# KamilSJaron/smudgeplot

Measured on NVIDIA H100. Metric: k-mers/sec scanned (hetmers) at 1/2/4/8 H100; bit-exact .smu vs ref C, higher is better.
Workload: dtype u64

## Files before the change

smudgeplot_b200/csrc/hm_symm.cu:

```cuda
#include <cuda_runtime.h>
#include <stdint.h>
#include <stdio.h>
#include <stdlib.h>
#include <string.h>

#include "hetmers_b200.h"
#include "hm_internal.h"
#include "hm_device.cuh"

#define RS_THREADS 256
#define RS_EPT     8
#define RS_TILE    (RS_THREADS*RS_EPT)
#define RS_HALO    64
#define RS_WIN     (RS_TILE+2*RS_HALO)
#define RS_SCANCAP RS_HALO
#define RS_RUNCAP  (RS_HALO+1)
#define RS_LONGRUN 32
#ifndef RS_MINBLOCKS
#define RS_MINBLOCKS 5
#endif
#ifndef RS_STAGE
#define RS_STAGE   384
#endif

#define SY_STATUS_ASYMMETRIC 1ull
#define SY_STATUS_OVERFLOW   2ull

#define SY_HDR_CAND   0
#define SY_HDR_STATUS 1
#define SY_HDR_RUNS   2
#define SY_HDR_S      3
#define SY_HDR_PEND   4
#define SY_HDR_QUERY  5

struct SymmView
  { unsigned long long *cand_n;
    unsigned long long *status;
    uint32_t *bloom;
    uint32_t  seg_words;
    int       n_seg, self;
    uint64_t  first_key[HM_MAX_SHARDS];
    uint64_t *cand_key, *cand_lo, *cand_meta;
    unsigned long long cand_cap;
    unsigned long long *runs_n;
    uint64_t *runs;
    unsigned long long runs_cap;
    uint64_t *s_key, *s_lo;
    unsigned long long s_cap;
    const hm_stream_sview *sviews;
    uint64_t *pend, *pend_key, *pend_lo;
    uint64_t *q_key, *q_lo, *q_tag;
    unsigned long long pend_cap, q_cap;
  };

template <int KW>
__device__ __forceinline__ void bloom_slot(const SymmView &W, int seg, int kmer, uint64_t hi, uint64_t lo,
                                           uint32_t *&word, uint32_t &mask)
{ const int Pr = kmer >> 1, pup = kmer-Pr;
  uint64_t sfx;
  if (KW == 1)
    sfx = hi >> (64-2*kmer);
  else
    { const int sr = 128-2*kmer;
      sfx = sr == 0 ? lo : ((lo >> sr) | (hi << (64-sr)));
    }
  if (2*Pr < 64)
    sfx &= (((uint64_t) 1 << (2*Pr)) - 1);
  const uint64_t pfx = hi >> (64-2*pup);
  uint32_t h = ((uint32_t) sfx ^ (uint32_t) (sfx >> 32) * 0x85EBCA6Bu) * 0x9E3779B1u;
  uint32_t g = ((uint32_t) pfx ^ (uint32_t) (pfx >> 32) * 0xC2B2AE35u) * 0x27D4EB2Fu;
  h ^= h >> 15;
  word = W.bloom + (size_t) seg * W.seg_words + __umulhi(h * 0x2C1B3C6Du,W.seg_words);
  mask = (1u << (g >> 27)) | (1u << ((g >> 22) & 31));
}

__device__ __forceinline__ uint32_t ld_keep(const uint32_t *p)
{ uint32_t v; uint64_t pol;
  asm volatile("createpolicy.fractional.L2::evict_last.b64 %0, 1.0;" : "=l"(pol));
  asm volatile("ld.global.nc.L1::no_allocate.L2::cache_hint.u32 %0, [%1], %2;" : "=r"(v) : "l"(p), "l"(pol));
  return v;
}

__device__ __forceinline__ uint64_t ld_stream(const uint64_t *p)
{ uint64_t v, pol;
  asm volatile("createpolicy.fractional.L2::evict_first.b64 %0, 1.0;" : "=l"(pol));
  asm volatile("ld.global.nc.L1::no_allocate.L2::cache_hint.u64 %0, [%1], %2;" : "=l"(v) : "l"(p), "l"(pol));
  return v;
}

__device__ __forceinline__ int owner_of(const SymmView &W, uint64_t hi)
{ int r = 0;
  for (int s = 1; s < W.n_seg; s++)
    r += (hi >= W.first_key[s]);
  return r;
}

template <typename IdxT, int KW>
__device__ __noinline__ void neighbours_slow(const uint64_t *__restrict__ keys, const uint64_t *__restrict__ keys_lo,
                                             const uint16_t *__restrict__ cnt, const IdxT *__restrict__ bucket,
                                             int bshift, int kmer, int p0, int pup,
                                             uint64_t x, uint64_t xl, int cx,
                                             int &H, int &U, int64_t &part, int &ppos)
{ H = 0; U = 0; part = -1; ppos = 0;
  for (int p = p0; p < kmer; p++)
    { int b = base_at<KW>(x,xl,p);
      for (int c = 0; c < 4; c++)
        { if (c == b) continue;
          uint64_t y = x, yl = xl;
          set_base<KW>(y,yl,p,c);
          int64_t j = bucket_find<IdxT,KW>(keys,keys_lo,bucket,bshift,y,yl);
          if (j >= 0 && cx + (int) __ldg(cnt+j) <= HM_SMAX)
            { H += 1;
              if (p >= pup) U += 1;
              part = j; ppos = p;
            }
        }
    }
}


__device__ __forceinline__ uint64_t fp_mix(uint64_t hi, uint64_t lo, uint32_t c, uint64_t seed)
{ uint64_t v = (hi ^ seed) * 0xBF58476D1CE4E5B9ull;
  v ^= v >> 32;
  v = (v + lo + ((uint64_t) c << 40) + c) * 0x94D049BB133111EBull;
  v ^= v >> 29;
  v *= (seed | 1);
  v ^= v >> 32;
  return v;
}

template <int KW>
__global__ void __launch_bounds__(256)
symm_fingerprint_kernel(const uint64_t *__restrict__ keys, const uint64_t *__restrict__ keys_lo,
                        const uint16_t *__restrict__ cnt, int64_t i0, int64_t i1, int kmer,
                        uint64_t seed0, uint64_t seed1, unsigned long long *__restrict__ acc)
{ uint64_t a0 = 0, a1 = 0, a2 = 0, a3 = 0;
  const int64_t stride = (int64_t) gridDim.x * blockDim.x;
  for (int64_t i = i0 + (int64_t) blockIdx.x * blockDim.x + threadIdx.x; i < i1; i += stride)
    { uint64_t x = keys[i], xl = KW == 2 ? keys_lo[i] : 0, r, rl;
      uint32_t c = cnt[i];
      revcomp_kmer<KW>(x,xl,kmer,r,rl);
      a0 += fp_mix(x,xl,c,seed0);  a1 += fp_mix(x,xl,c,seed1);
      a2 += fp_mix(r,rl,c,seed0);  a3 += fp_mix(r,rl,c,seed1);
    }
  for (int o = 16; o > 0; o >>= 1)
    { a0 += __shfl_xor_sync(0xffffffffu,a0,o); a1 += __shfl_xor_sync(0xffffffffu,a1,o);
      a2 += __shfl_xor_sync(0xffffffffu,a2,o); a3 += __shfl_xor_sync(0xffffffffu,a3,o);
    }
  if ((threadIdx.x & 31) == 0)
    { atomicAdd(acc+0,(unsigned long long) a0); atomicAdd(acc+1,(unsigned long long) a1);
      atomicAdd(acc+2,(unsigned long long) a2); atomicAdd(acc+3,(unsigned long long) a3);
    }
}

extern "C" int hm_k_symm_fingerprint(const uint64_t *d_keys, const uint64_t *d_keys_lo, const uint16_t *d_cnt,
                                     int64_t i0, int64_t i1, int kmer, const uint64_t seed[2],
                                     uint64_t *d_acc, void *stream)
{ if (kmer < 1 || kmer > HM_MAX_KMER || (kmer > 32) != (d_keys_lo != NULL) || seed == NULL || d_acc == NULL)
    return hm_set_error(HM_EINVAL,"symm_fingerprint: bad arguments (k=%d)",kmer);
  if (i1 <= i0)
    return HM_OK;
  int64_t want = (i1-i0+255)/256;
  int     grid = (int) (want < 132*16 ? want : 132*16);
  if (kmer <= 32)
    symm_fingerprint_kernel<1><<<grid,256,0,(cudaStream_t) stream>>>
        (d_keys,NULL,d_cnt,i0,i1,kmer,seed[0],seed[1],(unsigned long long *) d_acc);
  else
    symm_fingerprint_kernel<2><<<grid,256,0,(cudaStream_t) stream>>>
        (d_keys,d_keys_lo,d_cnt,i0,i1,kmer,seed[0],seed[1],(unsigned long long *) d_acc);
  cudaError_t e = cudaGetLastError();
  if (e != cudaSuccess)
    return hm_cuda_fail(e,"symm_fingerprint_kernel");
  return HM_OK;
}

extern "C" void hm_symm_seeds(uint64_t seed[2])
// ... 236 lines not shown
                      int Hy, Uy, py; int64_t party;
                      neighbours_slow<IdxT,KW>(keys,keys_lo,cnt,bucket,bshift,kmer,Pr,pup,y,yl,cy,Hy,Uy,party,py);
                      if (Hy == 1)
                        { emit = true;
                          meta = pack_meta(cx,cy,ppos,base_at<KW>(y,yl,ppos));
                        }
                    }
                }
              const unsigned eb = __ballot_sync(FULL,emit);
              if (eb != 0)
                { unsigned long long base = 0;
                  if (lane == 0)
                    base = atomicAdd(W.cand_n,(unsigned long long) __popc(eb));
                  base = __shfl_sync(FULL,base,0) + (unsigned long long) __popc(eb & lt);
                  if (emit)
                    { if (base < W.cand_cap)
                        { W.cand_key[base] = x;
                          if (KW == 2) W.cand_lo[base] = xl;
                          W.cand_meta[base] = meta;
                        }
                      else
                        atomicOr(W.status,SY_STATUS_OVERFLOW);
                    }
                }
            }
        }
    }
}

template <int KW> struct RunSfx    { typedef uint64_t T; };
template <>       struct RunSfx<1> { typedef uint32_t T; };

template <int KW>
__device__ __forceinline__ typename RunSfx<KW>::T run_sfx(uint64_t hi, uint64_t lo, int Pr)
{ if constexpr (KW == 1)
    return (uint32_t) ((hi << 2*Pr) >> 32);
  else
    return (hi << (2*Pr-32) << 32) | (lo >> (64-2*Pr));
}

template <typename T>
__device__ __forceinline__ bool one_base_in_run(T d, int Pr, int &pos)
{ const T u = (d | (d >> 1)) & (T) HM_M5;
  if constexpr (sizeof(T) == 4) pos = Pr + (__clz((int) d) >> 1);
  else                          pos = Pr + (__clzll((long long) d) >> 1);
  return (u & (u-1)) == 0;
}

template <int KW, bool SL, int LMAX>
__device__ __forceinline__ bool settle_members(const RsSmem<KW> &S, const SymmView &W, int kmer, int Pr, int pup,
                                               int h, int L, int a, bool in, bool own, int lane,
                                               uint64_t &x, uint64_t &xl, uint64_t &meta)
{ int Hx = 0, Ux = 0, part = 0, ppos = 0, cx = 0;
  if (in)
    { x  = S.key[h+a];
      xl = KW == 2 ? S.klo[h+a] : 0;
      cx = S.cnt[h+a];
      auto mate = [&](int b)
        { int pos;
          if (b < L && b != a && one_base_in_run(run_sfx<KW>(x ^ S.key[h+b],KW == 2 ? xl ^ S.klo[h+b] : 0,Pr),Pr,pos) &&
              cx + (int) S.cnt[h+b] <= HM_SMAX)
            { Hx += 1;
              if (pos >= pup) Ux += 1;
              part = b; ppos = pos;
            }
        };
      if constexpr (LMAX > 0)
        {
#pragma unroll
          for (int b = 0; b < LMAX; b++)
            mate(b);
        }
      else
        for (int b = 0; b < L; b++)
          mate(b);
      if (own && Ux > 0)
        bloom_insert<KW,SL>(W,kmer,x,xl);
    }
  const int pl = lane + part - a;
  int       Hy = __shfl_sync(0xffffffffu,Hx,pl & 31);
  if (!in || !own || Hx != 1 || part < a)
    return false;
  const uint64_t y = S.key[h+part], yl = KW == 2 ? S.klo[h+part] : 0;
  const int      cy = S.cnt[h+part];
  if (pl > 31)
    { Hy = 0;
      for (int b = 0; b < L; b++)
        { int pos;
          if (b != part && one_base_in_run(run_sfx<KW>(y ^ S.key[h+b],KW == 2 ? yl ^ S.klo[h+b] : 0,Pr),Pr,pos) &&
              cy + (int) S.cnt[h+b] <= HM_SMAX)
            Hy += 1;
        }
    }
  if (Hy != 1)
    return false;
  meta = pack_meta(cx,cy,ppos,base_at<KW>(y,yl,ppos));
  return true;
}

#ifdef RS_PROBE
#define RS_PHASES 6
#define RS_PROBE_SLOTS 1024
__device__ unsigned long long rs_probe_cycles[RS_PROBE_SLOTS*RS_PHASES];
__device__ int rs_probe_mode;
#define RS_PROBE_TILE(b)  (rs_probe_mode == 2 ? (b) % 64 : (b))
#define RS_PROBE_START    long long rs_t = clock64(); unsigned long long rs_acc[RS_PHASES] = {0, 0, 0, 0, 0, 0};
#define RS_PROBE_MARK(ph) { const long long t_ = clock64(); rs_acc[ph] += (unsigned long long) (t_ - rs_t); rs_t = t_; }
#define RS_PROBE_FLUSH()  { if (lane == 0) _Pragma("unroll") for (int p_ = 0; p_ < RS_PHASES; p_++) \
                              atomicAdd(rs_probe_cycles + (blockIdx.x % RS_PROBE_SLOTS)*RS_PHASES + p_,rs_acc[p_]); }
#define RS_PROBE_LOADONLY() if (rs_probe_mode == 1) { RS_PROBE_FLUSH(); return; }

extern "C" int hm_probe_runscan(int mode, unsigned long long *cycles)
{ static unsigned long long rows[RS_PROBE_SLOTS*RS_PHASES];
  cudaError_t e = cudaDeviceSynchronize();
  if (e == cudaSuccess && cycles != NULL)
    { e = cudaMemcpyFromSymbol(rows,rs_probe_cycles,sizeof(rows));
      for (int p = 0; p < RS_PHASES; p++)
        { cycles[p] = 0;
          for (int r = 0; r < RS_PROBE_SLOTS; r++)
            cycles[p] += rows[r*RS_PHASES+p];
        }
    }
  memset(rows,0,sizeof(rows));
  if (e == cudaSuccess)
    e = cudaMemcpyToSymbol(rs_probe_cycles,rows,sizeof(rows));
  if (e == cudaSuccess)
    e = cudaMemcpyToSymbol(rs_probe_mode,&mode,sizeof(mode));
  return e == cudaSuccess ? HM_OK : hm_cuda_fail(e,"hm_probe_runscan");
}
#else
#define RS_PROBE_TILE(b)  (b)
#define RS_PROBE_START
#define RS_PROBE_MARK(ph)
#define RS_PROBE_FLUSH()
#define RS_PROBE_LOADONLY()
#endif

template <typename IdxT, int KW, bool SL>
__global__ void __launch_bounds__(RS_THREADS,RS_MINBLOCKS)
runscan_kernel(const uint64_t *__restrict__ keys, const uint64_t *__restrict__ keys_lo,
               const uint16_t *__restrict__ cnt, int64_t n, const IdxT *__restrict__ bucket, int bshift,
               int kmer, int64_t lo, int64_t hi, int64_t tile0, int use_tma, const SymmView W)
{ extern __shared__ __align__(128) uint8_t smem[];
  __shared__ __align__(8) uint64_t s_bar;
  __shared__ unsigned s_nc, s_nr, s_done;
  RsSmem<KW> S;
  S.key   = (uint64_t *) smem;
  S.klo   = S.key + (KW == 2 ? RS_WIN : 0);
  S.ckey  = S.key + KW*RS_WIN;
  S.clo   = S.ckey + (KW == 2 ? RS_STAGE : 0);
  S.cmeta = S.ckey + KW*RS_STAGE;
  S.cnt   = (uint16_t *) (S.cmeta + RS_STAGE);
  S.t1    = S.cnt + RS_WIN;
  S.t2r   = S.t1 + RS_TILE/2;

  const int      Pr   = kmer >> 1;
  const int      pup  = kmer - Pr;
  const int      psh  = 64-2*Pr;
  const uint64_t pmask = ~(uint64_t) 0 << psh;
  const unsigned FULL = 0xffffffffu;
  const int      lane = threadIdx.x & 31;
  const int      warp = threadIdx.x >> 5;
  const unsigned lt   = (1u << lane) - 1;
  RS_PROBE_START

  const int64_t T0 = (tile0 + RS_PROBE_TILE(blockIdx.x)) * RS_TILE;
  const int64_t ws = T0 - RS_HALO;
  const int64_t e0 = ws > 0 ? ws : 0;
  const int64_t e1 = T0+RS_TILE+RS_HALO < n ? T0+RS_TILE+RS_HALO : n;
  const int     v0 = (int) (e0-ws), v1 = (int) (e1-ws);

  const int m   = v1-v0;
  const int mt  = use_tma ? (m & ~7) : 0;
  if (threadIdx.x == 0)
    { s_nc = 0; s_nr = 0; s_done = 0;
      if (mt > 0)
        { mbar_init(&s_bar,1);
          fence_proxy_async_smem();
        }
    }
  __syncthreads();
  if (threadIdx.x == 0 && mt > 0)
    { mbar_arrive_expect_tx(&s_bar,(unsigned) (mt*(8*KW+2)));
      bulk_copy_g2s(S.key+v0,keys+e0,(unsigned) (8*mt),&s_bar);
      if (KW == 2)
        bulk_copy_g2s(S.klo+v0,keys_lo+e0,(unsigned) (8*mt),&s_bar);
      bulk_copy_g2s(S.cnt+v0,cnt+e0,(unsigned) (2*mt),&s_bar);
    }
  if (mt < m || v0 > 0 || v1 < RS_WIN)
    { for (int j = mt + threadIdx.x; j < m; j += RS_THREADS)
        { S.key[v0+j] = keys[e0+j];
          if (KW == 2) S.klo[v0+j] = keys_lo[e0+j];
          S.cnt[v0+j] = cnt[e0+j];
        }
      if (mt > 0)
        mbar_wait(&s_bar,0);
      __syncthreads();
      const uint64_t sa = ~S.key[v0], sb = ~S.key[v1-1];
      __syncthreads();
      for (int j = threadIdx.x; j < RS_WIN; j += RS_THREADS)
        if (j < v0)       S.key[j] = sa;
        else if (j >= v1) S.key[j] = sb;
      __syncthreads();
    }
  else
    mbar_wait(&s_bar,0);
  RS_PROBE_MARK(0)
  RS_PROBE_LOADONLY()

  const int wd0 = RS_HALO/32 + warp*RS_EPT;
  unsigned  eqw = 0;
#pragma unroll
  for (int t = 0; t < RS_EPT+2; t++)
    { const int i = (wd0-1+t)*32 + lane;
      bool eq;
      if (psh >= 32)
        { const uint32_t a = (uint32_t) (S.key[i] >> 32);
          uint32_t       b = __shfl_down_sync(FULL,a,1);
          if (lane == 31) b = (uint32_t) (S.key[i+1] >> 32);
          eq = (((a ^ b) >> (psh-32)) == 0);
        }
      else
        eq = (((S.key[i] ^ S.key[i+1]) & pmask) == 0);
      const unsigned bal = __ballot_sync(FULL,eq);
      if (lane == t) eqw = bal;
    }
  RS_PROBE_MARK(1)

  const int a0 = RS_HALO + (lo > T0 ? (int) (lo-T0 < RS_TILE ? lo-T0 : RS_TILE) : 0);
  const int a1 = RS_HALO + (hi-T0 < RS_TILE ? (int) (hi-T0) : RS_TILE);
  uint16_t *my1  = S.t1  + warp*(RS_TILE/2/(RS_THREADS/32));
  int n1, n3;
  { const unsigned P = __shfl_up_sync(FULL,eqw,1), N = __shfl_down_sync(FULL,eqw,1);
    unsigned m2 = 0, m3 = 0;
    const int wd = wd0-1+lane;
    if (lane >= 1 && lane <= RS_EPT)
      { const unsigned E = eqw;
        const unsigned em1 = (E << 1) | (P >> 31);
        const unsigned em2 = (E << 2) | (P >> 30);
        const unsigned ep1 = (E >> 1) | (N << 31);
        const int      s0  = wd*32;
        unsigned act = 0xffffffffu;
        if (s0 < a0)      act &= (a0-s0 >= 32) ? 0u : (0xffffffffu << (a0-s0));
        if (s0+32 > a1)   act &= (a1-s0 <= 0)  ? 0u : (0xffffffffu >> (s0+32-a1));
        const unsigned more = (em1 & E) | (E & ep1) | (em1 & em2);
        m2 = (E & ~em1 & ~ep1) & act;
        m3 = more & act & ~em1;
      }
    const int c2 = __popc(m2), c3 = __popc(m3);
    int pre2 = c2, pre3 = c3;
#pragma unroll
    for (int o = 1; o <= RS_EPT; o <<= 1)
      { int v2 = __shfl_up_sync(FULL,pre2,o), v3 = __shfl_up_sync(FULL,pre3,o);
        if (lane >= o) { pre2 += v2; pre3 += v3; }
      }
    n1 = __shfl_sync(FULL,pre2,RS_EPT);
    n3 = __shfl_sync(FULL,pre3,RS_EPT);
    int at = pre2-c2;
    while (m2 != 0)
      { my1[at++] = (uint16_t) (wd*32 + __ffs(m2)-1);
        m2 &= m2-1;
      }
    at = n1 + pre3-c3;
    while (m3 != 0)
      { my1[at++] = (uint16_t) (wd*32 + __ffs(m3)-1);
        m3 &= m3-1;
      }
  }
  __syncwarp();
  RS_PROBE_MARK(2)

  for (int i0 = 0; i0 < n1; i0 += 32)
    { const int i = i0+lane;
      bool     emit = false;
      uint64_t x = 0, xl = 0, meta = 0;
      if (i < n1)
        { const int w = my1[i];
          x = S.key[w];
          const uint64_t y = S.key[w+1];
          uint64_t yl = 0;
          if (KW == 2) { xl = S.klo[w]; yl = S.klo[w+1]; }
          const int cx = S.cnt[w], cy = S.cnt[w+1];
          int pos;
          if (one_base_in_run(run_sfx<KW>(x ^ y,xl ^ yl,Pr),Pr,pos) && cx+cy <= HM_SMAX)
            { emit = true;
              meta = pack_meta(cx,cy,pos,base_at<KW>(y,yl,pos));
              if (pos >= pup)
                { bloom_insert<KW,SL>(W,kmer,x,xl);
                  bloom_insert<KW,SL>(W,kmer,y,yl);
                }
            }
        }
      stage_candidates<KW>(S,&s_nc,W,emit,x,xl,meta,lane,lt);
    }
  RS_PROBE_MARK(3)

  const int b1 = hi-T0 < RS_TILE+RS_HALO ? RS_HALO + (int) (hi-T0) : RS_WIN;
  for (int i0 = 0; i0 < n3; i0 += 32)
    { const int i = i0+lane;
      const int h = i < n3 ? my1[n1+i] : 0;
      int       L = 0;
      {
        const int      t  = (h >> 5) - (wd0-1);
        const unsigned w0 = __shfl_sync(FULL,eqw,t & 31), w1 = __shfl_sync(FULL,eqw,(t+1) & 31);
        const unsigned up = __funnelshift_r(w0,w1,h & 31);
        if (i < n3)
          L = (~up != 0) ? __ffs((int) ~up) : 33;
      }
      const int Ls = L <= 8 ? L : 0;
      int inc = Ls;
#pragma unroll
      for (int o = 1; o < 32; o <<= 1)
        { const int v = __shfl_up_sync(FULL,inc,o);
          if (lane >= o) inc += v;
        }
      const int M = __shfl_sync(FULL,inc,31);
      for (int t0 = 0; t0 < M; t0 += 32)
        { const int t = t0+lane;
          int r = 0;
#pragma unroll
          for (int s = 16; s > 0; s >>= 1)
            if (__shfl_sync(FULL,inc,r+s-1) <= t) r += s;
          const int hr = __shfl_sync(FULL,h,r), Lr = __shfl_sync(FULL,Ls,r);
          const int a  = t - (__shfl_sync(FULL,inc,r) - Lr);
          bool     emit = false;
          uint64_t x = 0, xl = 0, meta = 0;
          emit = settle_members<KW,SL,8>(S,W,kmer,Pr,pup,hr,Lr,a,t < M,hr+a < b1,lane,x,xl,meta);
          stage_candidates<KW>(S,&s_nc,W,emit,x,xl,meta,lane,lt);
        }
      unsigned lb = __ballot_sync(FULL,L > 8);
      while (lb != 0)
        { const int src = __ffs(lb)-1;
          lb &= lb-1;
          const int hh = __shfl_sync(FULL,h,src);
          int       LL = __shfl_sync(FULL,L,src);
          if (LL > 32)
            { const uint64_t xh = S.key[hh];
              while (LL <= RS_RUNCAP)
                { const int      t = hh+LL+lane;
                  const unsigned sb = __ballot_sync(FULL,t < RS_WIN && ((S.key[t] ^ xh) & pmask) == 0);
                  if (sb != FULL) { LL += __ffs(~sb)-1; break; }
                  LL += 32;
                }
            }
          if (LL > RS_RUNCAP || hh+LL >= RS_WIN)
            { if (lane == 0)
                S.t2r[atomicAdd(&s_nr,1u)] = (uint16_t) hh;
              continue;
            }
          for (int a0 = 0; a0 < LL; a0 += 32)
            { const int a = a0+lane;
              bool     emit = false;
              uint64_t x = 0, xl = 0, meta = 0;
              emit = settle_members<KW,SL,0>(S,W,kmer,Pr,pup,hh,LL,a,a < LL,hh+a < b1,lane,x,xl,meta);
              stage_candidates<KW>(S,&s_nc,W,emit,x,xl,meta,lane,lt);
            }
        }
    }
  RS_PROBE_MARK(4)

  __syncwarp();
  unsigned last = 0;
  if (lane == 0)
    { __threadfence_block();
      last = (atomicAdd(&s_done,1u) == RS_THREADS/32-1);
    }
  last = __shfl_sync(FULL,last,0);
  if (!last)
    { RS_PROBE_MARK(5) RS_PROBE_FLUSH() return; }
  __threadfence_block();
  const unsigned nr = s_nr;
  if (nr > 0)
    { unsigned long long rb = 0;
      if (lane == 0)
        rb = atomicAdd(W.runs_n,(unsigned long long) nr);
      rb = __shfl_sync(FULL,rb,0);
      for (unsigned i = lane; i < nr; i += 32)
        if (rb+i < W.runs_cap)
          W.runs[rb+i] = (uint64_t) (T0 + ((int) S.t2r[i] - RS_HALO));
        else
          atomicOr(W.status,SY_STATUS_OVERFLOW);
    }
  const unsigned nc = s_nc < RS_STAGE ? s_nc : RS_STAGE;
  if (nc == 0)
    { RS_PROBE_MARK(5) RS_PROBE_FLUSH() return; }
  unsigned long long base = 0;
  if (lane == 0)
    base = atomicAdd(W.cand_n,(unsigned long long) nc);
  base = __shfl_sync(FULL,base,0);
  for (unsigned i = lane; i < nc; i += 32)
    { unsigned long long at = base + i;
      if (at < W.cand_cap)
        { W.cand_key[at] = S.ckey[i];
          if (KW == 2) W.cand_lo[at] = S.clo[i];
          W.cand_meta[at] = S.cmeta[i];
        }
      else
        atomicOr(W.status,SY_STATUS_OVERFLOW);
    }
  RS_PROBE_MARK(5)
  RS_PROBE_FLUSH()
}

template <typename IdxT, int KW, bool SL>
__global__ void __launch_bounds__(RS_THREADS,RS_MINBLOCKS)
runscan_dense_kernel(const uint64_t *__restrict__ keys, const uint64_t *__restrict__ keys_lo,
                     const uint16_t *__restrict__ cnt, int64_t n, int kmer, int64_t lo, int64_t hi,
                     int64_t tile0, int use_tma, const SymmView W)
{ extern __shared__ __align__(128) uint8_t smem[];
  __shared__ __align__(8) uint64_t s_bar;
  __shared__ unsigned s_nc, s_nl, s_done;
  __shared__ unsigned s_eq[RS_WIN/32+1];
  RsSmem<KW> S;
  S.key   = (uint64_t *) smem;
  S.klo   = S.key + (KW == 2 ? RS_WIN : 0);
  S.ckey  = S.key + KW*RS_WIN;
  S.clo   = S.ckey + (KW == 2 ? RS_STAGE : 0);
  S.cmeta = S.ckey + KW*RS_STAGE;
  S.cnt   = (uint16_t *) (S.cmeta + RS_STAGE);
  S.t1    = S.cnt + RS_WIN;
  S.t2r   = S.t1 + RS_WIN;
  uint16_t *s_part = S.t2r + RS_TILE/8;
  unsigned *hu = (unsigned *) (s_part + RS_WIN);
  uint32_t *rem = hu + RS_WIN/2;

  const int      Pr   = kmer >> 1, pup = kmer - Pr, psh = 64-2*Pr;
  const uint64_t pmask = ~(uint64_t) 0 << psh;
  const unsigned FULL = 0xffffffffu;
  const int      lane = threadIdx.x & 31;
  const int      warp = threadIdx.x >> 5;
  const unsigned lt   = (1u << lane) - 1;

  const int64_t T0 = (tile0 + blockIdx.x) * RS_TILE;
  const int64_t ws = T0 - RS_HALO;
  const int64_t e0 = ws > 0 ? ws : 0;
  const int64_t e1 = T0+RS_TILE+RS_HALO < n ? T0+RS_TILE+RS_HALO : n;
  const int     v0 = (int) (e0-ws), v1 = (int) (e1-ws);

  const int m   = v1-v0;
  const int mt  = use_tma ? (m & ~7) : 0;
  if (threadIdx.x == 0)
    { s_nc = 0; s_nl = 0; s_done = 0;
      if (mt > 0)
        { mbar_init(&s_bar,1);
          fence_proxy_async_smem();
        }
    }
  for (int j = threadIdx.x; j < RS_WIN/2; j += RS_THREADS)
    hu[j] = 0;
  __syncthreads();
  if (threadIdx.x == 0 && mt > 0)
    { mbar_arrive_expect_tx(&s_bar,(unsigned) (mt*(8*KW+2)));
      bulk_copy_g2s(S.key+v0,keys+e0,(unsigned) (8*mt),&s_bar);
      if (KW == 2)
        bulk_copy_g2s(S.klo+v0,keys_lo+e0,(unsigned) (8*mt),&s_bar);
      bulk_copy_g2s(S.cnt+v0,cnt+e0,(unsigned) (2*mt),&s_bar);
    }
  if (mt < m || v0 > 0 || v1 < RS_WIN)
    { for (int j = mt + threadIdx.x; j < m; j += RS_THREADS)
        { S.key[v0+j] = keys[e0+j];
          if (KW == 2) S.klo[v0+j] = keys_lo[e0+j];
          S.cnt[v0+j] = cnt[e0+j];
        }
      if (mt > 0)
        mbar_wait(&s_bar,0);
      __syncthreads();
      const uint64_t sa = ~S.key[v0], sb = ~S.key[v1-1];
      __syncthreads();
      for (int j = threadIdx.x; j < RS_WIN; j += RS_THREADS)
        if (j < v0)       S.key[j] = sa;
        else if (j >= v1) S.key[j] = sb;
      __syncthreads();
    }
  else
    mbar_wait(&s_bar,0);

  const bool narrow = (KW == 1) && (kmer-Pr <= 16);
  for (int wd = warp; wd < RS_WIN/32; wd += RS_THREADS/32)
    { const int i = wd*32 + lane;
      bool eq = false;
      const uint64_t ki = S.key[i];
      if (i+1 < RS_WIN)
        eq = (((ki ^ S.key[i+1]) & pmask) == 0);
// ... 20 lines not shown
          back = (~dn == 0) ? 32 : __clz((int) ~dn);
        }
      uint16_t mark = (uint16_t) fwd;
      if (back+fwd+1 > RS_LONGRUN)
        { mark = 0xffff;
          if (back == 0 && i >= a0 && i < a1)
            S.t2r[atomicAdd(&s_nl,1u)] = (uint16_t) i;
        }
      S.t1[i] = mark;
      s_part[i] = (uint16_t) i;
    }
  __syncthreads();

  for (int i = threadIdx.x; i < RS_WIN; i += RS_THREADS)
    { const int fwd = S.t1[i];
      if (fwd == 0 || fwd == 0xffff)
        continue;
      const int cx = S.cnt[i];
      if (narrow)
        { const uint32_t rx = rem[i];
          for (int j = i+1; j <= i+fwd; j++)
            { const uint32_t d = rx ^ rem[j];
              const uint32_t u = (d | (d>>1)) & 0x55555555u;
              if ((u & (u-1)) == 0 && cx + (int) S.cnt[j] <= HM_SMAX)
                { const int      pos = Pr + (__clz((int) d) >> 1);
                  const unsigned inc = 1u | (pos >= pup ? 0x100u : 0u);
                  atomicAdd(hu + (i>>1), inc << (16*(i&1)));
                  atomicAdd(hu + (j>>1), inc << (16*(j&1)));
                  s_part[i] = (uint16_t) j;
                  s_part[j] = (uint16_t) i;
                }
            }
        }
      else
        { const uint64_t x = S.key[i], xl = KW == 2 ? S.klo[i] : 0;
          for (int j = i+1; j <= i+fwd; j++)
            { int pos;
              if (one_base_apart<KW>(x,xl,S.key[j],KW == 2 ? S.klo[j] : 0,pos) && cx + (int) S.cnt[j] <= HM_SMAX)
                { const unsigned inc = 1u | (pos >= pup ? 0x100u : 0u);
                  atomicAdd(hu + (i>>1), inc << (16*(i&1)));
                  atomicAdd(hu + (j>>1), inc << (16*(j&1)));
                  s_part[i] = (uint16_t) j;
                  s_part[j] = (uint16_t) i;
                }
            }
        }
    }
  __syncthreads();

  for (int i0 = RS_HALO + (threadIdx.x & ~31); i0 < RS_HALO+RS_TILE; i0 += RS_THREADS)
    { const int i = i0+lane;
      bool     emit = false;
      uint64_t x = 0, xl = 0, meta = 0;
      if (i >= a0 && i < a1 && S.t1[i] != 0xffff)
        { const unsigned c = (hu[i>>1] >> (16*(i&1))) & 0xffffu;
          const int H = (int) (c & 0xff), U = (int) (c >> 8);
          if (H > 0)
            { x = S.key[i];
              if (KW == 2) xl = S.klo[i];
              if (U > 0)
                bloom_insert<KW,SL>(W,kmer,x,xl);
              const int j = s_part[i];
              if (H == 1 && j > i && ((hu[j>>1] >> (16*(j&1))) & 0xffu) == 1)
                { const uint64_t y = S.key[j], yl = KW == 2 ? S.klo[j] : 0;
                  int pos;
                  one_base_apart<KW>(x,xl,y,yl,pos);
                  emit = true;
                  meta = pack_meta(S.cnt[i],S.cnt[j],pos,base_at<KW>(y,yl,pos));
                }
            }
        }
      stage_candidates<KW>(S,&s_nc,W,emit,x,xl,meta,lane,lt);
    }

  __syncwarp();
  unsigned last = 0;
  if (lane == 0)
    { __threadfence_block();
      last = (atomicAdd(&s_done,1u) == RS_THREADS/32-1);
    }
  last = __shfl_sync(FULL,last,0);
  if (!last)
    return;
  __threadfence_block();
  const unsigned nr = s_nl;
  if (nr > 0)
    { unsigned long long rb = 0;
      if (lane == 0)
        rb = atomicAdd(W.runs_n,(unsigned long long) nr);
      rb = __shfl_sync(FULL,rb,0);
      for (unsigned i = lane; i < nr; i += 32)
        if (rb+i < W.runs_cap)
          W.runs[rb+i] = (uint64_t) (T0 + ((int) S.t2r[i] - RS_HALO));
        else
          atomicOr(W.status,SY_STATUS_OVERFLOW);
    }
  const unsigned nc = s_nc < RS_STAGE ? s_nc : RS_STAGE;
  if (nc == 0)
    return;
  unsigned long long base = 0;
  if (lane == 0)
    base = atomicAdd(W.cand_n,(unsigned long long) nc);
  base = __shfl_sync(FULL,base,0);
  for (unsigned i = lane; i < nc; i += 32)
    { unsigned long long at = base + i;
      if (at < W.cand_cap)
        { W.cand_key[at] = S.ckey[i];
          if (KW == 2) W.cand_lo[at] = S.clo[i];
          W.cand_meta[at] = S.cmeta[i];
        }
      else
        atomicOr(W.status,SY_STATUS_OVERFLOW);
    }
}

template <typename I, int K> struct Inst { typedef I IdxT; static constexpr int KW = K; };

template <class F>
static cudaError_t dispatch(int kmer, int idx64, F f)
{ if (kmer <= 32)
    return idx64 ? f(Inst<uint64_t,1>()) : f(Inst<uint32_t,1>());
  return idx64 ? f(Inst<uint64_t,2>()) : f(Inst<uint32_t,2>());
}

template <typename IdxT, int KW, bool SL = false>
static cudaError_t launch_runscan(const uint64_t *keys, const uint64_t *keys_lo, const uint16_t *cnt, int64_t n,
                                  const void *bucket, int bits, int kmer, int64_t lo, int64_t hi,
                                  const SymmView &W, cudaStream_t st)
{ static int configured[64] = {0};
  int dev = 0;
  cudaGetDevice(&dev);
  int64_t tile0 = lo/RS_TILE, tile1 = (hi+RS_TILE-1)/RS_TILE;
  int     tma   = ((((uintptr_t) keys) | ((uintptr_t) cnt) | ((uintptr_t) (keys_lo ? keys_lo : keys))) & 15) == 0;
  const int   Pr  = kmer >> 1;
  double      lam = (2*Pr >= 62) ? 0.0 : (double) n / (double) ((uint64_t) 1 << (2*Pr));
  bool        dense = (lam > 0.6);
  const char *force = getenv("HETMERS_RUNSCAN");
  if (force != NULL && strcmp(force,"dense") == 0)  dense = true;
  if (force != NULL && strcmp(force,"sparse") == 0) dense = false;
  cudaError_t e;
  if (dense)
    { size_t smem = (size_t) RS_WIN*(8*KW+2) + (size_t) RS_STAGE*8*(KW+1) +
                    2*(size_t) (RS_WIN+RS_TILE/8+RS_WIN) + 4*(size_t) (RS_WIN/2+RS_WIN);
      if (smem > 48*1024 && (dev >= 64 || !(configured[dev] & 2)))
        { e = cudaFuncSetAttribute(runscan_dense_kernel<IdxT,KW,SL>,cudaFuncAttributeMaxDynamicSharedMemorySize,(int) smem);
          if (e != cudaSuccess) return e;
          if (dev < 64) configured[dev] |= 2;
        }
      runscan_dense_kernel<IdxT,KW,SL><<<(unsigned) (tile1-tile0),RS_THREADS,smem,st>>>
          (keys,keys_lo,cnt,n,kmer,lo,hi,tile0,tma,W);
    }
  else
    { size_t smem = (size_t) RS_WIN*(8*KW+2) + (size_t) RS_STAGE*8*(KW+1) +
                    2*(size_t) (RS_TILE/2+RS_TILE/2);
      if (smem > 48*1024 && (dev >= 64 || !(configured[dev] & 1)))
        { e = cudaFuncSetAttribute(runscan_kernel<IdxT,KW,SL>,cudaFuncAttributeMaxDynamicSharedMemorySize,(int) smem);
          if (e != cudaSuccess) return e;
          if (dev < 64) configured[dev] |= 1;
        }
      runscan_kernel<IdxT,KW,SL><<<(unsigned) (tile1-tile0),RS_THREADS,smem,st>>>
          (keys,keys_lo,cnt,n,(const IdxT *) bucket,64-bits,kmer,lo,hi,tile0,tma,W);
    }
  return cudaGetLastError();
}

template <typename IdxT, int KW, bool SL = false>
static cudaError_t launch_runs(const uint64_t *keys, const uint64_t *keys_lo, const uint16_t *cnt, int64_t n,
                               const void *bucket, int bits, int kmer, int64_t lo, int64_t hi,
                               const SymmView &W, cudaStream_t st)
{
  int dev = 0, sms = 132;
  cudaGetDevice(&dev);
  cudaDeviceGetAttribute(&sms,cudaDevAttrMultiProcessorCount,dev);
  int64_t want = ((hi-lo)/64+255)/256;
  int     grid = (int) (want < sms*8 ? (want > 0 ? want : 1) : sms*8);
  runs_kernel<IdxT,KW,SL><<<grid,256,0,st>>>(keys,keys_lo,cnt,n,(const IdxT *) bucket,64-bits,kmer,lo,hi,W);
  return cudaGetLastError();
}

extern "C" int hm_k_symm_runscan(const uint64_t *d_keys, const uint64_t *d_keys_lo, const uint16_t *d_cnt, int64_t n,
                                 const void *d_bucket, int bits, int idx64, int kmer, int64_t lo, int64_t hi,
                                 void *d_work, const hm_symm_layout *layout, const hm_symm_shards *shards,
                                 void *stream)
{ if (kmer < HM_SYMM_MIN_KMER || kmer > HM_MAX_KMER)
    return hm_set_error(HM_EUNSUPPORTED,"symmetric scan needs %d <= k <= %d (k=%d)",HM_SYMM_MIN_KMER,HM_MAX_KMER,kmer);
  if (lo < 0 || hi > n || lo > hi || bits < 1 || bits > 30 || d_work == NULL || layout == NULL)
    return hm_set_error(HM_EINVAL,"symm_runscan: bad range [%lld,%lld) of %lld or bits %d",
                        (long long) lo,(long long) hi,(long long) n,bits);
  if ((kmer > 32) != (d_keys_lo != NULL))
    return hm_set_error(HM_EINVAL,"symm_runscan: second key word array %s for k=%d",
                        d_keys_lo ? "given" : "missing",kmer);
  if ((shards != NULL && shards->n_seg > 1) != (layout->n_seg > 1) ||
      (shards != NULL && shards->n_seg > 1 && (shards->n_seg != layout->n_seg || shards->self < 0 ||
                                               shards->self >= shards->n_seg)))
    return hm_set_error(HM_EINVAL,"symm_runscan: shard table does not match the work-area layout");
  cudaStream_t st = (cudaStream_t) stream;
  SymmView W = make_view(d_work,layout,shards);
  HM_CUDA(cudaMemsetAsync(W.cand_n,0,256,st));
  HM_CUDA(cudaMemsetAsync(W.bloom + (size_t) W.self*W.seg_words,0,sizeof(uint32_t)*(size_t) W.seg_words,st));
  if (l2_persist())
    bloom_window(st,W.bloom,sizeof(uint32_t)*(size_t) W.seg_words*(size_t) W.n_seg,1);
  if (hi == lo)
    return HM_OK;
  cudaError_t e = dispatch(kmer,idx64,[&](auto I)
    { return launch_runscan<typename decltype(I)::IdxT,decltype(I)::KW>(d_keys,d_keys_lo,d_cnt,n,d_bucket,bits,kmer,
                                                                       lo,hi,W,st); });
  if (e != cudaSuccess)
    return hm_cuda_fail(e,"runscan_kernel");
  return HM_OK;
}

extern "C" int hm_k_symm_runs(const uint64_t *d_keys, const uint64_t *d_keys_lo, const uint16_t *d_cnt, int64_t n,
                              const void *d_bucket, int bits, int idx64, int kmer, int64_t lo, int64_t hi,
                              void *d_work, const hm_symm_layout *layout, const hm_symm_shards *shards,
                              void *stream)
{ if (kmer < HM_SYMM_MIN_KMER || kmer > HM_MAX_KMER || d_work == NULL || layout == NULL ||
      (kmer > 32) != (d_keys_lo != NULL) || lo < 0 || hi > n || lo > hi)
    return hm_set_error(HM_EINVAL,"symm_runs: bad arguments");
  if (hi == lo)
    return HM_OK;
  cudaStream_t st = (cudaStream_t) stream;
  SymmView W = make_view(d_work,layout,shards);
  cudaError_t e = dispatch(kmer,idx64,[&](auto I)
    { return launch_runs<typename decltype(I)::IdxT,decltype(I)::KW>(d_keys,d_keys_lo,d_cnt,n,d_bucket,bits,kmer,
                                                                    lo,hi,W,st); });
  if (e != cudaSuccess)
    return hm_cuda_fail(e,"runs_kernel");
  return HM_OK;
}


#define RV_TS   192
#define RV_TM   96
#define RV_TROW 97
#define RV_THREADS 1024
#ifndef RV_ILP
#define RV_ILP 2
#endif
#define RV_QCAP  (32*(RV_ILP+1))
#define RV_PROBE 4
#define RV_HA    (1ull << 48)
#define RV_HB    (1ull << 49)

#ifdef RESOLVE_PROBE
#define RVP_BINS 50
#define RVP_CAND 0
#define RVP_HA   1
#define RVP_HB   2
#define RVP_HAB  3
#define RVP_GEN  4
#define RVP_HIST 5
#define RVP_NCTR (RVP_HIST+RVP_BINS)
__device__ unsigned long long rvp_ctr[RVP_NCTR];
__device__ int rvp_mode;
#define RVP_MODE rvp_mode
#define RVP_COUNT(i,v) { if (rvp_mode == 3) atomicAdd(rvp_ctr+(i),(unsigned long long) (v)); }
#define RVP_BUCKET(sz) RVP_COUNT(RVP_HIST + ((sz) < RVP_BINS-1 ? (int) (sz) : RVP_BINS-1),1)

extern "C" int hm_probe_resolve(int mode, unsigned long long *ctr)
{ static unsigned long long rows[RVP_NCTR];
  cudaError_t e = cudaDeviceSynchronize();
  if (e == cudaSuccess && ctr != NULL)
    { e = cudaMemcpyFromSymbol(rows,rvp_ctr,sizeof(rows));
      memcpy(ctr,rows,sizeof(rows));
    }
  memset(rows,0,sizeof(rows));
  if (e == cudaSuccess)
    e = cudaMemcpyToSymbol(rvp_ctr,rows,sizeof(rows));
  if (e == cudaSuccess)
    e = cudaMemcpyToSymbol(rvp_mode,&mode,sizeof(mode));
  return e == cudaSuccess ? HM_OK : hm_cuda_fail(e,"hm_probe_resolve");
}
#else
#define RVP_MODE 0
#define RVP_COUNT(i,v)
#define RVP_BUCKET(sz)
#endif

template <int KW>
__device__ __forceinline__ bool bucket_upper_partner(const uint64_t *__restrict__ keys, const uint64_t *__restrict__ keys_lo,
                                                     const uint16_t *__restrict__ cnt, int64_t l, int64_t r,
                                                     int psh, int pup, uint64_t q, uint64_t ql, int cq, bool &found)
{ bool hit = false;
  found = false;
  for (int64_t i0 = l; i0 < r; i0 += RV_PROBE)
    { uint64_t z[RV_PROBE];
#pragma unroll
      for (int u = 0; u < RV_PROBE; u++)
        z[u] = (i0+u < r) ? __ldg(keys+i0+u) : ~q;
#pragma unroll
      for (int u = 0; u < RV_PROBE; u++)
        { if (((z[u] ^ q) >> psh) != 0)
            continue;
          const uint64_t zl = KW == 2 ? __ldg(keys_lo+i0+u) : 0;
          int pos;
          if (z[u] == q && (KW == 1 || zl == ql))
            found = true;
          else if (one_base_apart<KW>(q,ql,z[u],zl,pos) && pos >= pup && cq + (int) __ldg(cnt+i0+u) <= HM_SMAX)
            hit = true;
        }
    }
  return hit;
}

template <typename IdxT, int KW>
__device__ __noinline__ bool has_upper_partner(const uint64_t *__restrict__ keys, const uint64_t *__restrict__ keys_lo,
                                               const uint16_t *__restrict__ cnt, int64_t n,
// ... 815 lines not shown
```

Before: 119.4 billion.

## Classify short runs by bitmask and emit members directly, skipping warp scan expansion

Run heads are now split with bit tricks into short runs (length at most 8) and long runs. Short runs have all their member positions written straight into the per-warp list through an add-carry fill mask, and each member recovers its run start and length from the eq bitmask with funnel shifts and clz/ffs. This removes the per-batch warp prefix scan and binary search that previously expanded short runs into members. Long runs are stored from the end of an enlarged per-warp list, the three counts are packed into one scan, and the list shared memory grows a little, which could affect occupancy.

```diff
diff --git a/smudgeplot_b200/csrc/hm_symm.cu b/smudgeplot_b200/csrc/hm_symm.cu
--- a/smudgeplot_b200/csrc/hm_symm.cu
+++ b/smudgeplot_b200/csrc/hm_symm.cu
@@ -22,6 +22,7 @@
 #ifndef RS_STAGE
 #define RS_STAGE   384
 #endif
+#define RS_WLIST   (RS_TILE/(RS_THREADS/32)+8)
 
 #define SY_STATUS_ASYMMETRIC 1ull
 #define SY_STATUS_OVERFLOW   2ull
@@ -564,7 +565,7 @@
   S.cmeta = S.ckey + KW*RS_STAGE;
   S.cnt   = (uint16_t *) (S.cmeta + RS_STAGE);
   S.t1    = S.cnt + RS_WIN;
-  S.t2r   = S.t1 + RS_TILE/2;
+  S.t2r   = S.t1 + RS_WLIST*(RS_THREADS/32);
 
   const int      Pr   = kmer >> 1;
   const int      pup  = kmer - Pr;
@@ -641,43 +642,54 @@
 
   const int a0 = RS_HALO + (lo > T0 ? (int) (lo-T0 < RS_TILE ? lo-T0 : RS_TILE) : 0);
   const int a1 = RS_HALO + (hi-T0 < RS_TILE ? (int) (hi-T0) : RS_TILE);
-  uint16_t *my1  = S.t1  + warp*(RS_TILE/2/(RS_THREADS/32));
-  int n1, n3;
+  uint16_t *my1  = S.t1  + warp*RS_WLIST;
+  int n1, nm, n9;
   { const unsigned P = __shfl_up_sync(FULL,eqw,1), N = __shfl_down_sync(FULL,eqw,1);
-    unsigned m2 = 0, m3 = 0;
-    const int wd = wd0-1+lane;
+    unsigned m2 = 0, m9 = 0, mlo = 0, mhi = 0;
     if (lane >= 1 && lane <= RS_EPT)
       { const unsigned E = eqw;
         const unsigned em1 = (E << 1) | (P >> 31);
         const unsigned em2 = (E << 2) | (P >> 30);
         const unsigned ep1 = (E >> 1) | (N << 31);
-        const int      s0  = wd*32;
+        const int      s0  = (wd0-1+lane)*32;
         unsigned act = 0xffffffffu;
         if (s0 < a0)      act &= (a0-s0 >= 32) ? 0u : (0xffffffffu << (a0-s0));
         if (s0+32 > a1)   act &= (a1-s0 <= 0)  ? 0u : (0xffffffffu >> (s0+32-a1));
         const unsigned more = (em1 & E) | (E & ep1) | (em1 & em2);
         m2 = (E & ~em1 & ~ep1) & act;
-        m3 = more & act & ~em1;
+        const unsigned m3 = more & act & ~em1;
+        const uint64_t X  = (uint64_t) E | ((uint64_t) N << 32);
+        uint64_t       c8 = X & (X >> 1);
+        c8 &= c8 >> 2;
+        c8 &= c8 >> 4;
+        m9 = m3 & (uint32_t) c8;
+        const uint64_t fill = (X + (m3 & ~(uint32_t) c8)) ^ X;
+        mlo = (uint32_t) fill;
+        mhi = (uint32_t) (fill >> 32);
       }
-    const int c2 = __popc(m2), c3 = __popc(m3);
-    int pre2 = c2, pre3 = c3;
+    const unsigned mm = mlo | __shfl_up_sync(FULL,mhi,1);
+    const unsigned c = __popc(m2) | (__popc(mm) << 10) | (__popc(m9) << 20);
+    unsigned pre = c;
 #pragma unroll
     for (int o = 1; o <= RS_EPT; o <<= 1)
-      { int v2 = __shfl_up_sync(FULL,pre2,o), v3 = __shfl_up_sync(FULL,pre3,o);
-        if (lane >= o) { pre2 += v2; pre3 += v3; }
+      { const unsigned v = __shfl_up_sync(FULL,pre,o);
+        if (lane >= o) pre += v;
       }
-    n1 = __shfl_sync(FULL,pre2,RS_EPT);
-    n3 = __shfl_sync(FULL,pre3,RS_EPT);
-    int at = pre2-c2;
-    while (m2 != 0)
-      { my1[at++] = (uint16_t) (wd*32 + __ffs(m2)-1);
-        m2 &= m2-1;
-      }
-    at = n1 + pre3-c3;
-    while (m3 != 0)
-      { my1[at++] = (uint16_t) (wd*32 + __ffs(m3)-1);
-        m3 &= m3-1;
-      }
+    const unsigned tot = __shfl_sync(FULL,pre,RS_EPT+1);
+    n1 = tot & 1023;
+    nm = (tot >> 10) & 1023;
+    n9 = tot >> 20;
+    pre -= c;
+    const int s0 = (wd0-1+lane)*32;
+    int at = pre & 1023;
+    for (unsigned b = m2; b != 0; b &= b-1)
+      my1[at++] = (uint16_t) (s0 + __ffs(b)-1);
+    at = n1 + ((pre >> 10) & 1023);
+    for (unsigned b = mm; b != 0; b &= b-1)
+      my1[at++] = (uint16_t) (s0 + __ffs(b)-1);
+    at = RS_WLIST-1 - (int) (pre >> 20);
+    for (unsigned b = m9; b != 0; b &= b-1)
+      my1[at--] = (uint16_t) (s0 + __ffs(b)-1);
   }
   __syncwarp();
   RS_PROBE_MARK(2)
@@ -708,39 +720,32 @@
   RS_PROBE_MARK(3)
 
   const int b1 = hi-T0 < RS_TILE+RS_HALO ? RS_HALO + (int) (hi-T0) : RS_WIN;
-  for (int i0 = 0; i0 < n3; i0 += 32)
+  for (int i0 = 0; i0 < nm; i0 += 32)
+    { const int      i  = i0+lane;
+      const int      s  = i < nm ? my1[n1+i] : wd0*32;
+      const int      tq = ((s-1) >> 5) - (wd0-1), ts = (s >> 5) - (wd0-1);
+      const unsigned q0 = __shfl_sync(FULL,eqw,(tq-1) & 31), q1 = __shfl_sync(FULL,eqw,tq & 31);
+      const unsigned w0 = __shfl_sync(FULL,eqw,ts & 31),     w1 = __shfl_sync(FULL,eqw,(ts+1) & 31);
+      const unsigned dn = __funnelshift_l(q0,q1,31-((s-1) & 31));
+      const unsigned up = __funnelshift_r(w0,w1,s & 31);
+      const int      a  = __clz((int) ~dn), L = a + __ffs((int) ~up);
+      bool     emit = false;
+      uint64_t x = 0, xl = 0, meta = 0;
+      emit = settle_members<KW,SL,8>(S,W,kmer,Pr,pup,s-a,L,a,i < nm,s < b1,lane,x,xl,meta);
+      stage_candidates<KW>(S,&s_nc,W,emit,x,xl,meta,lane,lt);
+    }
+  for (int i0 = 0; i0 < n9; i0 += 32)
     { const int i = i0+lane;
-      const int h = i < n3 ? my1[n1+i] : 0;
+      const int h = i < n9 ? my1[RS_WLIST-1-i] : 0;
       int       L = 0;
       {
         const int      t  = (h >> 5) - (wd0-1);
         const unsigned w0 = __shfl_sync(FULL,eqw,t & 31), w1 = __shfl_sync(FULL,eqw,(t+1) & 31);
         const unsigned up = __funnelshift_r(w0,w1,h & 31);
-        if (i < n3)
+        if (i < n9)
           L = (~up != 0) ? __ffs((int) ~up) : 33;
       }
-      const int Ls = L <= 8 ? L : 0;
-      int inc = Ls;
-#pragma unroll
-      for (int o = 1; o < 32; o <<= 1)
-        { const int v = __shfl_up_sync(FULL,inc,o);
-          if (lane >= o) inc += v;
-        }
-      const int M = __shfl_sync(FULL,inc,31);
-      for (int t0 = 0; t0 < M; t0 += 32)
-        { const int t = t0+lane;
-          int r = 0;
-#pragma unroll
-          for (int s = 16; s > 0; s >>= 1)
-            if (__shfl_sync(FULL,inc,r+s-1) <= t) r += s;
-          const int hr = __shfl_sync(FULL,h,r), Lr = __shfl_sync(FULL,Ls,r);
-          const int a  = t - (__shfl_sync(FULL,inc,r) - Lr);
-          bool     emit = false;
-          uint64_t x = 0, xl = 0, meta = 0;
-          emit = settle_members<KW,SL,8>(S,W,kmer,Pr,pup,hr,Lr,a,t < M,hr+a < b1,lane,x,xl,meta);
-          stage_candidates<KW>(S,&s_nc,W,emit,x,xl,meta,lane,lt);
-        }
-      unsigned lb = __ballot_sync(FULL,L > 8);
+      unsigned lb = __ballot_sync(FULL,i < n9);
       while (lb != 0)
         { const int src = __ffs(lb)-1;
           lb &= lb-1;
@@ -1067,7 +1072,7 @@
     }
   else
     { size_t smem = (size_t) RS_WIN*(8*KW+2) + (size_t) RS_STAGE*8*(KW+1) +
-                    2*(size_t) (RS_TILE/2+RS_TILE/2);
+                    2*(size_t) (RS_WLIST*(RS_THREADS/32)+RS_TILE/2);
       if (smem > 48*1024 && (dev >= 64 || !(configured[dev] & 1)))
         { e = cudaFuncSetAttribute(runscan_kernel<IdxT,KW,SL>,cudaFuncAttributeMaxDynamicSharedMemorySize,(int) smem);
           if (e != cudaSuccess) return e;
```

Result: no change. 119.8 billion, median of 6 (+0.3%).
